# lesliegaga/GPT-SoVITS

Hardware: AMD Instinct MI355X
Metric: synthesised audio sec/sec (1/RTF), v2 pipeline (higher is better)
Workload: dtype f16

## Files before the change

### gpt-sovits_amd/csrc/conv_pair.hip

```cpp
#include <stdlib.h>

#include <algorithm>

#include "common.h"

namespace gsv {

namespace {

typedef _Float16 T;
typedef h8 F;
typedef _Float16 T4 __attribute__((ext_vector_type(4)));

__device__ __forceinline__ void mma32p(f16v& acc, const h8& a, const h8& b) { acc = __builtin_amdgcn_mfma_f32_32x32x16_f16(a, b, acc, 0, 0, 0); }
__device__ __forceinline__ h8 lrelu8(h8 v, float s) { h8 t = v * (_Float16)s; return __builtin_elementwise_max(v, t); }
__device__ __forceinline__ T4 lrelu4(T4 v, float s) { T4 t = v * (_Float16)s; return __builtin_elementwise_max(v, t); }

constexpr int ROWS_Y = 288;
constexpr int ROWS_X = 338;

template <int CC, int TAPS, bool ACCU>
__global__ __launch_bounds__(256, CC == 32 ? 2 : 3) void conv_pair_f16_kernel(ConvPairArgs a, int ntiles) {
  constexpr int G = 8, KC = 16, CT = 32, WN = 4, TN = 2, NT = 256;
  constexpr int LDX = CC + G, VPR = CC / G;
  constexpr int XB = (ROWS_X * VPR + NT - 1) / NT;
  constexpr int WPP = CC == 16 ? 2 : 4, NP = WN / WPP;
  constexpr int LDO = CT + 4, PR = TN * 32 * WPP, IPR = CT / 4, NI = PR * IPR / NT;
  extern __shared__ __attribute__((aligned(16))) unsigned char smem[];
  T* xs = (T*)smem;
  T* ys = xs + (size_t)ROWS_X * LDX;
  T* w2s = ys + (size_t)ROWS_Y * LDX;
  float* os = (float*)smem;
  static_assert(PR * LDO * 4 <= (ROWS_X + ROWS_Y) * LDX * 2, "epilogue tile must fit in window + intermediate image");
  const int tid = threadIdx.x, lane = tid & 63, wn = tid >> 6;
  const int r = lane & 31, h = lane >> 5;
  const T* __restrict__ x = a.x;
  const int h2 = (TAPS - 1) / 2, h1 = h2 * a.dil;
  const int rows_win = ROWS_Y + 2 * h1;
  const int total = rows_win * VPR;
  const int ecg = tid % IPR, ec = 4 * ecg;
  const int env = max(0, min(4, CC - ec));
  f4 ebias = (f4){0.f, 0.f, 0.f, 0.f};
  for (int j = 0; j < env; ++j) ebias[j] = a.b2[ec + j];
  f4 b1v[4];
#pragma unroll
  for (int g = 0; g < 4; ++g)
#pragma unroll
    for (int j = 0; j < 4; ++j) { const int c = 8 * g + 4 * h + j; b1v[g][j] = c < CC ? a.b1[c] : 0.f; }
  {
    const int totw = TAPS * CT * VPR;
    for (int v = tid; v < totw; v += NT) {
      const int tap = v / (CT * VPR), rem = v - tap * (CT * VPR);
      const int row = rem / VPR, col = rem - row * VPR;
      F val = {0, 0, 0, 0, 0, 0, 0, 0};
      if (row < CC) val = *(const F*)(a.w2 + (long long)row * TAPS * CC + (long long)tap * CC + col * G);
      *(F*)(w2s + ((size_t)tap * CT + row) * LDX + col * G) = val;
    }
  }
  F w1r[TAPS * (CC / KC)];
#pragma unroll
  for (int tap = 0; tap < TAPS; ++tap)
#pragma unroll
    for (int ks = 0; ks < CC / KC; ++ks) {
      F val = {0, 0, 0, 0, 0, 0, 0, 0};
      if (r < CC) val = *(const F*)(a.w1 + (long long)r * TAPS * CC + (long long)tap * CC + ks * KC + G * h);
      w1r[tap * (CC / KC) + ks] = val;
    }
  auto load_window = [&](int tile, F* regs) {
    const int win_start = tile * 256 - h2 - h1;
#pragma unroll
    for (int i = 0; i < XB; ++i) {
      const int v = min(tid + i * NT, total - 1);
      const int row = v / VPR, col = v - row * VPR;
      const int ti = win_start + row;
      const F val = *(const F*)(x + (long long)min(max(ti, 0), a.T - 1) * a.ldx + col * G);
      regs[i] = (ti >= 0 && ti < a.T) ? val : (F){0, 0, 0, 0, 0, 0, 0, 0};
    }
  };
  auto store_window = [&](const F* regs) {
#pragma unroll
    for (int i = 0; i < XB; ++i) {
      const int v = tid + i * NT;
      if (v < total) {
        const int row = v / VPR, col = v - row * VPR;
        *(F*)(xs + (size_t)row * LDX + col * G) = lrelu8(regs[i], 0.1f);
      }
    }
  };
  int tile = blockIdx.x;
  {
    F first[XB];
    load_window(min(tile, ntiles - 1), first);
    store_window(first);
  }
  __syncthreads();
  for (; tile < ntiles; tile += gridDim.x) {
    const int t0 = tile * 256;
    F nxt[XB];
    load_window(min(tile + (int)gridDim.x, ntiles - 1), nxt);
    T4 rv[NP * NI], yv[ACCU ? NP * NI : 1];
#pragma unroll
    for (int q = 0; q < NP * NI; ++q) {
      const int pass = q / NI, e = q - pass * NI;
      const int t = min(t0 + pass * PR + (tid + e * NT) / IPR, a.T - 1);
      const int cc = min(ec, CC - 4);
      rv[q] = *(const T4*)(x + (long long)t * a.ldx + cc);
      if (ACCU) yv[q] = *(const T4*)(a.y + (long long)t * a.ldy + cc);
    }
    for (int n1 = wn; n1 < ROWS_Y / 32; n1 += WN) {
      f16v acc;
#pragma unroll
      for (int i = 0; i < 16; ++i) acc[i] = 0.f;
#pragma unroll
      for (int tap = 0; tap < TAPS; ++tap) {
        const int shift = tap * a.dil;
#pragma unroll
        for (int ks = 0; ks < CC / KC; ++ks) {
          const int kk = ks * KC + G * h;
          const F bf = *(const F*)(xs + (size_t)(n1 * 32 + r + shift) * LDX + kk);
          mma32p(acc, w1r[tap * (CC / KC) + ks], bf);
        }
      }
      const int row = n1 * 32 + r, t = t0 - h2 + row;
      const bool inside = t >= 0 && t < a.T;
#pragma unroll
      for (int g = 0; g < 4; ++g) {
        const int c0 = 8 * g + 4 * h;
        if (c0 < CC) {
          T4 v = (T4){(T)(acc[4 * g] + b1v[g][0]), (T)(acc[4 * g + 1] + b1v[g][1]), (T)(acc[4 * g + 2] + b1v[g][2]),
                      (T)(acc[4 * g + 3] + b1v[g][3])};
          v = lrelu4(v, 0.1f);
          if (!inside) v = (T4){0, 0, 0, 0};
          *(T4*)(ys + (size_t)row * LDX + c0) = v;
        }
      }
    }
    __syncthreads();
    f16v acc2[TN];
#pragma unroll
    for (int n = 0; n < TN; ++n)
#pragma unroll
      for (int i = 0; i < 16; ++i) acc2[n][i] = 0.f;
    for (int tap = 0; tap < TAPS; ++tap) {
      const T* wb = w2s + (size_t)tap * CT * LDX;
#pragma unroll
      for (int ks = 0; ks < CC / KC; ++ks) {
        const int kk = ks * KC + G * h;
        const F af = *(const F*)(wb + (size_t)r * LDX + kk);
        F bf[TN];
#pragma unroll
        for (int n = 0; n < TN; ++n) bf[n] = *(const F*)(ys + (size_t)((wn * TN + n) * 32 + r + tap) * LDX + kk);
#pragma unroll
        for (int n = 0; n < TN; ++n) mma32p(acc2[n], af, bf[n]);
      }
    }
#pragma unroll
    for (int pass = 0; pass < NP; ++pass) {
      __syncthreads();
      if (wn / WPP == pass) {
#pragma unroll
        for (int n = 0; n < TN; ++n)
#pragma unroll
          for (int g = 0; g < 4; ++g)
            *(f4*)(os + (size_t)(((wn % WPP) * TN + n) * 32 + r) * LDO + 8 * g + 4 * h) =
                (f4){acc2[n][4 * g], acc2[n][4 * g + 1], acc2[n][4 * g + 2], acc2[n][4 * g + 3]};
      }
      __syncthreads();
#pragma unroll
      for (int e = 0; e < NI; ++e) {
        const int q = pass * NI + e;
        const int tl = (tid + e * NT) / IPR;
        const int t = t0 + pass * PR + tl;
        if (!(t < a.T && env > 0)) continue;
        const f4 av = *(const f4*)(os + (size_t)tl * LDO + 4 * ecg);
        float v[4];
#pragma unroll
        for (int j = 0; j < 4; ++j) {
          float u = av[j] + ebias[j];
          u += (float)rv[q][j];
          u *= a.scale;
          if (ACCU) u += (float)yv[q][j];
          v[j] = u;
        }
        T* yp = a.y + (long long)t * a.ldy + ec;
        if (env == 4) *(T4*)yp = (T4){(T)v[0], (T)v[1], (T)v[2], (T)v[3]};
        else for (int j = 0; j < env; ++j) yp[j] = (T)v[j];
      }
    }
    __syncthreads();
    store_window(nxt);
    __syncthreads();
  }
}

template <int CC, int TAPS>
int launch_pair(const ConvPairArgs& a, hipStream_t s) {
  const int ntiles = cdiv(a.T, 256);
  const size_t lds = ((size_t)ROWS_X + ROWS_Y + (size_t)TAPS * 32) * (CC + 8) * 2;
  static const int cap = getenv("GSV_PAIR_PER_CU") ? std::max(1, atoi(getenv("GSV_PAIR_PER_CU"))) : 3;
  const int per_cu = std::max(1, std::min(cap, (int)((156 * 1024) / lds)));
  const int grid = std::min(ntiles, 256 * per_cu);
#define GSV_PAIR(A)                                                                                                        \
  do {                                                                                                                     \
    auto kern = conv_pair_f16_kernel<CC, TAPS, A>;                                                                         \
    static bool set = false;                                                                                               \
    if (!set) { GSV_HIP(hipFuncSetAttribute((const void*)kern, hipFuncAttributeMaxDynamicSharedMemorySize, 160 * 1024)); set = true; } \
    hipLaunchKernelGGL(kern, dim3(grid), dim3(256), lds, s, a, ntiles);                                                    \
  } while (0)
  if (a.accumulate) GSV_PAIR(true);
  else GSV_PAIR(false);
#undef GSV_PAIR
  GSV_HIP(hipGetLastError());
  return GSV_OK;
}

template <int CC>
int launch_pair_taps(const ConvPairArgs& a, hipStream_t s) {
  switch (a.taps) {
    case 3: return launch_pair<CC, 3>(a, s);
    case 5: return launch_pair<CC, 5>(a, s);
    case 7: return launch_pair<CC, 7>(a, s);
    case 9: return launch_pair<CC, 9>(a, s);
    default: return launch_pair<CC, 11>(a, s);
  }
}

}

bool conv_pair_eligible(int dtype, int C, int taps, int dil, int T) {
  static const bool off = getenv("GSV_NO_CONV_PAIR") != nullptr;
  return !off && dtype == GSV_F16 && (C == 16 || C == 32) && (taps & 1) && taps <= 11 && dil >= 1 && ((taps - 1) / 2) * dil <= 25 &&
         T >= 256;
}

int launch_conv_pair(const ConvPairArgs& a, hipStream_t s) {
  GSV_REQUIRE(a.x && a.y && a.w1 && a.w2 && a.b1 && a.b2, "conv_pair: null operand");
  GSV_REQUIRE(conv_pair_eligible(GSV_F16, a.C, a.taps, a.dil, a.T) || getenv("GSV_NO_CONV_PAIR"), "conv_pair: shape C=%d taps=%d dil=%d T=%d not supported",
              a.C, a.taps, a.dil, a.T);
  GSV_REQUIRE(a.ldx % 8 == 0 && a.ldy % 4 == 0 && ((uintptr_t)a.x % 16) == 0 && ((uintptr_t)a.w1 % 16) == 0 && ((uintptr_t)a.w2 % 16) == 0,
              "conv_pair: operands must be 16-byte aligned");
  return a.C == 16 ? launch_pair_taps<16>(a, s) : launch_pair_taps<32>(a, s);
}

}
```

### gpt-sovits_amd/csrc/ops.hip

```cpp
#include "common.h"

namespace gsv {

static thread_local char g_err[1024] = "";
void set_error(const char* fmt, ...) {
  va_list ap;
  va_start(ap, fmt);
  vsnprintf(g_err, sizeof(g_err), fmt, ap);
  va_end(ap);
}
const char* get_error() { return g_err; }

template <typename T> __global__ void convert_kernel(const float* __restrict__ s, T* __restrict__ d, long long n) {
  long long i = (long long)blockIdx.x * blockDim.x + threadIdx.x;
  long long stride = (long long)gridDim.x * blockDim.x;
  for (; i < n; i += stride) d[i] = (T)s[i];
}

int launch_convert(const float* src, void* dst, int dtype, long long n, hipStream_t s) {
  if (n <= 0) return GSV_OK;
  int blocks = (int)((n + 255) / 256);
  if (blocks > 4096) blocks = 4096;
  if (dtype == GSV_F16) hipLaunchKernelGGL(convert_kernel<_Float16>, dim3(blocks), dim3(256), 0, s, src, (_Float16*)dst, n);
  else hipLaunchKernelGGL(convert_kernel<float>, dim3(blocks), dim3(256), 0, s, src, (float*)dst, n);
  GSV_HIP(hipGetLastError());
  return GSV_OK;
}

template <typename TX, typename TR, typename TY>
__global__ void layernorm_kernel(const TX* __restrict__ x, const TR* __restrict__ res, const float* __restrict__ gamma,
                                 const float* __restrict__ beta, TY* __restrict__ y, int rows, int C, float eps) {
  const int lane = threadIdx.x & 63;
  const int row = blockIdx.x * (blockDim.x >> 6) + (threadIdx.x >> 6);
  if (row >= rows) return;
  const TX* xr = x + (long long)row * C;
  const TR* rr = res ? res + (long long)row * C : nullptr;
  if (C <= 512) {
    float v[8];
    float s1 = 0.f;
#pragma unroll
    for (int i = 0; i < 8; ++i) {
      const int c = lane + 64 * i;
      v[i] = c < C ? to_f(xr[c]) + (rr ? to_f(rr[c]) : 0.f) : 0.f;
      s1 += v[i];
    }
    const float mean1 = wave_sum(s1) / (float)C;
    float q1 = 0.f;
#pragma unroll
    for (int i = 0; i < 8; ++i) {
      const float d = (lane + 64 * i < C) ? v[i] - mean1 : 0.f;
      q1 += d * d;
    }
    const float rstd1 = rsqrtf(wave_sum(q1) / (float)C + eps);
    TY* yr1 = y + (long long)row * C;
#pragma unroll
    for (int i = 0; i < 8; ++i) {
      const int c = lane + 64 * i;
      if (c < C) yr1[c] = (TY)((v[i] - mean1) * rstd1 * gamma[c] + beta[c]);
    }
    return;
  }
  float sum = 0.f;
  for (int c = lane; c < C; c += 64) sum += to_f(xr[c]) + (rr ? to_f(rr[c]) : 0.f);
  const float mean = wave_sum(sum) / (float)C;
  float var = 0.f;
  for (int c = lane; c < C; c += 64) {
    float d = to_f(xr[c]) + (rr ? to_f(rr[c]) : 0.f) - mean;
    var += d * d;
  }
  const float rstd = rsqrtf(wave_sum(var) / (float)C + eps);
  TY* yr = y + (long long)row * C;
  for (int c = lane; c < C; c += 64) {
    float v = to_f(xr[c]) + (rr ? to_f(rr[c]) : 0.f);
    yr[c] = (TY)((v - mean) * rstd * gamma[c] + beta[c]);
  }
}

template <typename TX, typename TR, typename TY>
static int ln_launch(const void* x, const void* res, const float* g, const float* b, void* y, int rows, int C, float eps,
                     hipStream_t s) {
  hipLaunchKernelGGL((layernorm_kernel<TX, TR, TY>), dim3(cdiv(rows, 4)), dim3(256), 0, s, (const TX*)x, (const TR*)res,
                     g, b, (TY*)y, rows, C, eps);
  GSV_HIP(hipGetLastError());
  return GSV_OK;
}

int launch_layernorm(int dtype, const void* x, int x_f32, const void* res, int res_f32, const float* gamma,
                     const float* beta, void* y, int y_f32, int rows, int C, float eps, hipStream_t s) {
  if (rows <= 0) return GSV_OK;
  const bool h = dtype == GSV_F16;
  const bool xf = x_f32 || !h, rf = res_f32 || !h, yf = y_f32 || !h;
  if (xf && rf && yf) return ln_launch<float, float, float>(x, res, gamma, beta, y, rows, C, eps, s);
  if (xf && rf && !yf) return ln_launch<float, float, _Float16>(x, res, gamma, beta, y, rows, C, eps, s);
  if (xf && !rf && !yf) return ln_launch<float, _Float16, _Float16>(x, res, gamma, beta, y, rows, C, eps, s);
  if (!xf && !rf && !yf) return ln_launch<_Float16, _Float16, _Float16>(x, res, gamma, beta, y, rows, C, eps, s);
  if (!xf && !rf && yf) return ln_launch<_Float16, _Float16, float>(x, res, gamma, beta, y, rows, C, eps, s);
  if (!xf && rf && !yf) return ln_launch<_Float16, float, _Float16>(x, res, gamma, beta, y, rows, C, eps, s);
  set_error("layernorm: unsupported dtype combination");
  return GSV_ERR_ARG;
}


template <typename T>
__global__ void frame_kernel(const float* __restrict__ x, int n, int flen, int hop, int pad, int ld, int T_out, T* __restrict__ out) {
  const int t = blockIdx.x;
  if (t >= T_out) return;
  for (int k = threadIdx.x; k < ld; k += blockDim.x) {
    float v = 0.f;
    if (k < flen) {
      int i = t * hop + k - pad;
      if (i < 0) i = -i;
      if (i >= n) i = 2 * (n - 1) - i;
      v = (i >= 0 && i < n) ? x[i] : 0.f;
    }
    out[(long long)t * ld + k] = (T)v;
  }
}

__global__ void magnitude_kernel(const float* __restrict__ ri, int T, int bins, float eps, float* __restrict__ spec) {
  __shared__ float tile[32][33];
  const int t0 = blockIdx.x * 32, b0 = blockIdx.y * 32;
  const int tx = threadIdx.x & 31, ty = threadIdx.x >> 5;
  for (int i = ty; i < 32; i += 8) {
    const int t = t0 + i, b = b0 + tx;
    float v = 0.f;
    if (t < T && b < bins) {
      const float re = ri[(long long)t * 2 * bins + b], im = ri[(long long)t * 2 * bins + bins + b];
      v = eps < 0.f ? re * re + im * im : sqrtf(re * re + im * im + eps);
    }
    tile[i][tx] = v;
  }
  __syncthreads();
  for (int i = ty; i < 32; i += 8) {
    const int b = b0 + i, t = t0 + tx;
    if (b < bins && t < T) spec[(long long)b * T + t] = tile[tx][i];
  }
}

__global__ void magnitude_tm_kernel(const float* __restrict__ ri, int T, int bins, int ld, float eps, float* __restrict__ spec) {
  const int b = blockIdx.x * 256 + threadIdx.x, t = blockIdx.y;
  if (b >= ld) return;
  float v = 0.f;
  if (b < bins) {
    const float re = ri[(long long)t * 2 * bins + b], im = ri[(long long)t * 2 * bins + bins + b];
    v = eps < 0.f ? re * re + im * im : sqrtf(re * re + im * im + eps);
  }
  spec[(long long)t * ld + b] = v;
}

__global__ void aff_mix_kernel(const float* __restrict__ x, const float* __restrict__ y, const float* __restrict__ t, long long n,
                               float* __restrict__ out) {
  const long long i = (long long)blockIdx.x * 256 + threadIdx.x;
  if (i < n) { const float a = t[i]; out[i] = x[i] * (1.f + a) + y[i] * (1.f - a); }
}

__global__ __launch_bounds__(1024) void time_mean_kernel(const float* __restrict__ x, int T, int ld, float* __restrict__ out) {
  __shared__ float part[16][64];
  const int c = blockIdx.x * 64 + (threadIdx.x & 63), sl = threadIdx.x >> 6;
  float s = 0.f;
  if (c < ld) for (int t = sl; t < T; t += 16) s += x[(long long)t * ld + c];
  part[sl][threadIdx.x & 63] = s;
  __syncthreads();
  if (sl == 0 && c < ld) {
    float v = 0.f;
    for (int k = 0; k < 16; ++k) v += part[k][threadIdx.x & 63];
    out[c] = v / (float)T;
  }
}

template <typename T>
__global__ void cnorm_stats_kernel(const T* __restrict__ x, int Tn, int C, int slices, float* __restrict__ part ) {
  const int c = blockIdx.x * blockDim.x + threadIdx.x, sl = blockIdx.y;
  if (c >= C) return;
  const int per = (Tn + slices - 1) / slices, t0 = sl * per, t1 = min(Tn, t0 + per);
  float s = 0.f, q = 0.f;
  for (int t = t0; t < t1; ++t) { const float v = to_f(x[(long long)t * C + c]); s += v; q += v * v; }
  part[((long long)sl * 2 + 0) * C + c] = s;
  part[((long long)sl * 2 + 1) * C + c] = q;
}
template <typename T>
__global__ void cnorm_apply_kernel(const T* __restrict__ x, int Tn, int C, int slices, const float* __restrict__ part,
                                   const float* __restrict__ gamma, const float* __restrict__ beta, float eps, int act, T* __restrict__ y) {
  const int c = blockIdx.x * blockDim.x + threadIdx.x;
  if (c >= C) return;
  double s = 0.0, q = 0.0;
  for (int sl = 0; sl < slices; ++sl) { s += part[((long long)sl * 2 + 0) * C + c]; q += part[((long long)sl * 2 + 1) * C + c]; }
  const float mean = (float)(s / Tn);
  const float var = fmaxf((float)(q / Tn - (s / Tn) * (s / Tn)), 0.f);
  const float a = rsqrtf(var + eps) * gamma[c], b = beta[c] - mean * a;
  const int per = (Tn + gridDim.y - 1) / gridDim.y, t0 = blockIdx.y * per, t1 = min(Tn, t0 + per);
  for (int t = t0; t < t1; ++t) y[(long long)t * C + c] = (T)post_act_f(act, to_f(x[(long long)t * C + c]) * a + b);
}

}

extern "C" {
const char* gsv_last_error(void) { return gsv::get_error(); }
int gsv_abi_version(void) { return 1; }
int gsv_init(int device) {
  int n = 0;
  hipError_t e = hipGetDeviceCount(&n);
  if (e != hipSuccess || n <= 0) {
    gsv::set_error("gsv_init: no HIP device (%s)", hipGetErrorString(e));
    return GSV_ERR_HIP;
  }
  if (device < 0 || device >= n) {
    gsv::set_error("gsv_init: device %d out of range (%d devices)", device, n);
    return GSV_ERR_ARG;
  }
  GSV_HIP(hipSetDevice(device));
  hipDeviceProp_t p;
  GSV_HIP(hipGetDeviceProperties(&p, device));
  if (strncmp(p.gcnArchName, "gfx950", 6) != 0) {
    gsv::set_error("gsv_init: device %d is %s, this library is built for gfx950 only", device, p.gcnArchName);
    return GSV_ERR_HIP;
  }
  return GSV_OK;
}

int gsv_op_layernorm(const void* x, const void* res, const float* gamma, const float* beta, void* y, int rows, int C,
                     float eps, int dtype, gsv_stream_t stream) {
  return gsv::launch_layernorm(dtype, x, 0, res, 0, gamma, beta, y, 0, rows, C, eps, (hipStream_t)stream);
}

int gsv_op_flash_attn64(const void* qkv, int T, int heads, float scale, void* vt_scratch, void* out, gsv_stream_t stream) {
  const int inner = heads * 64;
  return gsv::launch_flash_attn64_f16(qkv, 3 * inner, (const _Float16*)qkv + inner, 3 * inner, (const _Float16*)qkv + 2 * inner, 3 * inner,
                                      vt_scratch, T, heads, scale, out, inner, (hipStream_t)stream);
}

int gsv_op_flash_rel96(const void* qkv, int T, int heads, float scale, const float* rel_k, const float* rel_v, void* vt_scratch,
                       void* out, gsv_stream_t stream) {
  const int H = heads * 96;
  return gsv::launch_flash_rel96_f16(qkv, 3 * H, (const _Float16*)qkv + H, 3 * H, (const _Float16*)qkv + 2 * H, 3 * H, vt_scratch, T, heads,
                                     scale, rel_k, rel_v, out, H, (hipStream_t)stream);
}

int gsv_op_conv1d(const gsv_conv_desc* d, int dtype, gsv_stream_t stream) {
  gsv::ConvArgs a;
  a.x = d->x; a.w = d->w; a.bias = d->bias; a.y = d->y; a.res = d->res; a.gate = d->gate;
  a.T_in = d->T_in; a.T_out = d->T_out; a.Cin = d->Cin; a.Cout = d->Cout; a.taps = d->taps;
  a.stride = d->stride; a.dil = d->dil; a.pad = d->pad;
  a.ldx = d->Cin; a.ldw = d->taps * d->Cin;
  a.pre_act = d->pre_act; a.pre_slope = d->pre_slope; a.post_act = d->post_act; a.scale = d->scale;
  a.accumulate = d->accumulate; a.out_f32 = d->out_f32; a.res_f32 = d->out_f32;
  if (d->ups_u > 0) {
    a.ups_u = d->ups_u; a.ups_pad = d->ups_pad; a.ups_cout = d->Cout / d->ups_u;
    a.ldy = a.ups_cout; a.ldr = a.ups_cout;
    a.T_virt = d->T_in + d->taps - 1;
  } else {
    a.ldy = d->Cout; a.ldr = d->Cout;
    a.T_virt = d->T_out;
  }
  if (d->ldx > 0) a.ldx = d->ldx;
  if (d->ldw > 0) a.ldw = d->ldw;
  if (d->ldy > 0) { a.ldy = d->ldy; a.ldr = d->ldy; }
  if (d->ldr > 0) a.ldr = d->ldr;
  if (d->Z > 1) { a.Z = d->Z; a.xz = d->xz; a.wz = d->wz; a.yz = d->yz; a.bz = d->bz; a.rz = d->rz ? d->rz : d->yz; }
  return gsv::launch_conv_gemm(dtype, a, (hipStream_t)stream);
}

int gsv_op_frame(const float* x, int n, int frame_len, int hop, int pad, int ld, int T_out, void* out, int dtype, gsv_stream_t stream) {
  GSV_REQUIRE(x && out && n > 0 && frame_len > 0 && hop > 0 && ld >= frame_len && T_out > 0, "op_frame: bad argument");
  GSV_REQUIRE(pad >= 0 && pad < n, "op_frame: reflect padding %d needs more than %d samples", pad, pad);
  GSV_REQUIRE((long long)(T_out - 1) * hop + frame_len - pad <= (long long)n + pad, "op_frame: frames run past the (padded) signal");
  GSV_REQUIRE(dtype == GSV_F16 || dtype == GSV_F32, "op_frame: bad dtype");
  hipStream_t s = (hipStream_t)stream;
  if (dtype == GSV_F16) hipLaunchKernelGGL(gsv::frame_kernel<_Float16>, dim3(T_out), dim3(256), 0, s, x, n, frame_len, hop, pad, ld, T_out, (_Float16*)out);
  else hipLaunchKernelGGL(gsv::frame_kernel<float>, dim3(T_out), dim3(256), 0, s, x, n, frame_len, hop, pad, ld, T_out, (float*)out);
  GSV_HIP(hipGetLastError());
  return GSV_OK;
}

int gsv_op_magnitude(const float* re_im, int T, int bins, float eps, int frame_ld, float* spec, gsv_stream_t stream) {
  GSV_REQUIRE(re_im && spec && T > 0 && bins > 0, "op_magnitude: bad argument");
  GSV_REQUIRE(frame_ld == 0 || frame_ld >= bins, "op_magnitude: frame_ld %d is smaller than %d bins", frame_ld, bins);
  if (frame_ld == 0)
    hipLaunchKernelGGL(gsv::magnitude_kernel, dim3(gsv::cdiv(T, 32), gsv::cdiv(bins, 32)), dim3(256), 0, (hipStream_t)stream, re_im, T, bins, eps, spec);
  else
    hipLaunchKernelGGL(gsv::magnitude_tm_kernel, dim3(gsv::cdiv(frame_ld, 256), T), dim3(256), 0, (hipStream_t)stream, re_im, T, bins, frame_ld, eps, spec);
  GSV_HIP(hipGetLastError());
  return GSV_OK;
}

int gsv_op_conv_pair(const void* x, const void* w1, const float* b1, const void* w2, const float* b2, void* y, int T, int C, int taps,
                     int dil, float scale, int accumulate, gsv_stream_t stream) {
  GSV_REQUIRE(gsv::conv_pair_eligible(GSV_F16, C, taps, dil, T), "op_conv_pair: C must be 16 or 32, taps odd <= 11, (taps - 1) / 2 * dil <= 25, T >= 256");
  gsv::ConvPairArgs a;
  a.x = (const _Float16*)x; a.w1 = (const _Float16*)w1; a.b1 = b1; a.w2 = (const _Float16*)w2; a.b2 = b2; a.y = (_Float16*)y;
  a.T = T; a.C = C; a.taps = taps; a.dil = dil; a.ldx = C; a.ldy = C; a.scale = scale; a.accumulate = accumulate;
  return gsv::launch_conv_pair(a, (hipStream_t)stream);
}

int gsv_op_aff_mix(const float* x, const float* y, const float* t, long long n, float* out, gsv_stream_t stream) {
  GSV_REQUIRE(x && y && t && out && n > 0, "op_aff_mix: bad argument");
  hipLaunchKernelGGL(gsv::aff_mix_kernel, dim3((unsigned)((n + 255) / 256)), dim3(256), 0, (hipStream_t)stream, x, y, t, n, out);
  GSV_HIP(hipGetLastError());
  return GSV_OK;
}

int gsv_op_time_mean(const float* x, int T, int ld, float* out, gsv_stream_t stream) {
  GSV_REQUIRE(x && out && T > 0 && ld > 0, "op_time_mean: bad argument");
  hipLaunchKernelGGL(gsv::time_mean_kernel, dim3(gsv::cdiv(ld, 64)), dim3(1024), 0, (hipStream_t)stream, x, T, ld, out);
  GSV_HIP(hipGetLastError());
  return GSV_OK;
}

int gsv_op_channel_norm(const void* x, int T, int C, const float* gamma, const float* beta, float eps, int act, float* scratch,
                        void* y, int dtype, gsv_stream_t stream) {
  GSV_REQUIRE(x && y && gamma && beta && scratch && T > 0 && C > 0, "op_channel_norm: bad argument");
  GSV_REQUIRE(dtype == GSV_F16 || dtype == GSV_F32, "op_channel_norm: bad dtype");
  const int slices = 64;
  hipStream_t s = (hipStream_t)stream;
  const dim3 grid(gsv::cdiv(C, 64), slices);
  if (dtype == GSV_F16) {
    hipLaunchKernelGGL(gsv::cnorm_stats_kernel<_Float16>, grid, dim3(64), 0, s, (const _Float16*)x, T, C, slices, scratch);
    hipLaunchKernelGGL(gsv::cnorm_apply_kernel<_Float16>, grid, dim3(64), 0, s, (const _Float16*)x, T, C, slices, scratch, gamma, beta, eps, act, (_Float16*)y);
  } else {
    hipLaunchKernelGGL(gsv::cnorm_stats_kernel<float>, grid, dim3(64), 0, s, (const float*)x, T, C, slices, scratch);
    hipLaunchKernelGGL(gsv::cnorm_apply_kernel<float>, grid, dim3(64), 0, s, (const float*)x, T, C, slices, scratch, gamma, beta, eps, act, (float*)y);
  }
  GSV_HIP(hipGetLastError());
  return GSV_OK;
}
}
```

Measured before the change: 2782.

## Add fused conv-pair kernel for 64-channel HiFiGAN resblocks

Result: faster. 2817, median of 6 (+1.3%).

```diff
diff --git a/gpt-sovits_amd/csrc/conv_pair.hip b/gpt-sovits_amd/csrc/conv_pair.hip
--- a/gpt-sovits_amd/csrc/conv_pair.hip
+++ b/gpt-sovits_amd/csrc/conv_pair.hip
@@ -225,11 +225,237 @@
   }
 }
 
+constexpr int P64_TT = 128;
+constexpr int P64_RY = 160;
+constexpr int P64_RX = 210;
+
+template <int TAPS, int NW, bool ACCU>
+__global__ __launch_bounds__(64 * NW) void conv_pair64_f16_kernel(ConvPairArgs a, int ntiles) {
+  constexpr int CC = 64, G = 8, KC = 16, NT = 64 * NW, KS = CC / KC;
+  constexpr int WC = NW / 2, TN = 4 / WC;
+  constexpr int LDX = CC + G, VPR = CC / G;
+  constexpr int XB = (P64_RX * VPR + NT - 1) / NT;
+  constexpr int LDO = CC + 4, IPR = CC / 4, NI = P64_TT * IPR / NT;
+  static_assert(P64_TT * LDO * 4 <= (162 + P64_RY) * LDX * 2, "epilogue tile must fit in the smallest window + intermediate image");
+  extern __shared__ __attribute__((aligned(16))) unsigned char smem[];
+  const int h2 = (TAPS - 1) / 2, h1 = h2 * a.dil;
+  const int rows_win = P64_RY + 2 * h1;
+  T* xs = (T*)smem;
+  T* ys = xs + (size_t)rows_win * LDX;
+  T* w2s = ys + (size_t)P64_RY * LDX;
+  float* b1s = (float*)(w2s + (size_t)TAPS * CC * LDX);
+  float* os = (float*)smem;
+  const int tid = threadIdx.x, lane = tid & 63, wave = tid >> 6;
+  const int wm = wave & 1, wc = wave >> 1;
+  const int r = lane & 31, h = lane >> 5;
+  const T* __restrict__ x = a.x;
+  const int total = rows_win * VPR;
+  const int ecg = tid % IPR, ec = 4 * ecg;
+  f4 ebias;
+#pragma unroll
+  for (int j = 0; j < 4; ++j) ebias[j] = a.b2[ec + j];
+  {
+    const int totw = TAPS * CC * VPR;
+    for (int v = tid; v < totw; v += NT) {
+      const int tap = v / (CC * VPR), rem = v - tap * (CC * VPR);
+      const int row = rem / VPR, col = rem - row * VPR;
+      *(F*)(w2s + ((size_t)tap * CC + row) * LDX + col * G) = *(const F*)(a.w2 + (long long)row * TAPS * CC + (long long)tap * CC + col * G);
+    }
+    if (tid < CC) b1s[tid] = a.b1[tid];
+  }
+  F w1r[TAPS * KS];
+#pragma unroll
+  for (int tap = 0; tap < TAPS; ++tap)
+#pragma unroll
+    for (int ks = 0; ks < KS; ++ks)
+      w1r[tap * KS + ks] = *(const F*)(a.w1 + (long long)(wm * 32 + r) * TAPS * CC + (long long)tap * CC + ks * KC + G * h);
+  auto load_window = [&](int tile, F* regs) {
+    const int win_start = tile * P64_TT - h2 - h1;
+#pragma unroll
+    for (int i = 0; i < XB; ++i) {
+      const int v = min(tid + i * NT, total - 1);
+      const int row = v / VPR, col = v - row * VPR;
+      const int ti = win_start + row;
+      const F val = *(const F*)(x + (long long)min(max(ti, 0), a.T - 1) * a.ldx + col * G);
+      regs[i] = (ti >= 0 && ti < a.T) ? val : (F){0, 0, 0, 0, 0, 0, 0, 0};
+    }
+  };
+  auto store_window = [&](const F* regs) {
+#pragma unroll
+    for (int i = 0; i < XB; ++i) {
+      const int v = tid + i * NT;
+      if (v < total) {
+        const int row = v / VPR, col = v - row * VPR;
+        *(F*)(xs + (size_t)row * LDX + col * G) = lrelu8(regs[i], 0.1f);
+      }
+    }
+  };
+  int tile = blockIdx.x;
+  {
+    F first[XB];
+    load_window(min(tile, ntiles - 1), first);
+    store_window(first);
+  }
+  __syncthreads();
+  for (; tile < ntiles; tile += gridDim.x) {
+    const int t0 = tile * P64_TT;
+    F nxt[XB];
+    load_window(min(tile + (int)gridDim.x, ntiles - 1), nxt);
+    for (int n1 = wc; n1 < P64_RY / 32; n1 += WC) {
+      f16v acc;
+#pragma unroll
+      for (int i = 0; i < 16; ++i) acc[i] = 0.f;
+      const T* xb = xs + (size_t)(n1 * 32 + r) * LDX + G * h;
+      if constexpr (NW == 4) {
+        F bb[2][KS];
+#pragma unroll
+        for (int ks = 0; ks < KS; ++ks) bb[0][ks] = *(const F*)(xb + ks * KC);
+#pragma unroll
+        for (int tap = 0; tap < TAPS; ++tap) {
+          if (tap + 1 < TAPS) {
+#pragma unroll
+            for (int ks = 0; ks < KS; ++ks) bb[(tap + 1) & 1][ks] = *(const F*)(xb + (size_t)(tap + 1) * a.dil * LDX + ks * KC);
+          }
+          __builtin_amdgcn_sched_barrier(0);
+#pragma unroll
+          for (int ks = 0; ks < KS; ++ks) mma32p(acc, w1r[tap * KS + ks], bb[tap & 1][ks]);
+        }
+      } else {
+#pragma unroll
+        for (int tap = 0; tap < TAPS; ++tap) {
+          const int shift = tap * a.dil;
+#pragma unroll
+          for (int ks = 0; ks < KS; ++ks) mma32p(acc, w1r[tap * KS + ks], *(const F*)(xb + (size_t)shift * LDX + ks * KC));
+        }
+      }
+      const int row = n1 * 32 + r, t = t0 - h2 + row;
+      const bool inside = t >= 0 && t < a.T;
+#pragma unroll
+      for (int g = 0; g < 4; ++g) {
+        const int c0 = wm * 32 + 8 * g + 4 * h;
+        const f4 bv = *(const f4*)(b1s + c0);
+        T4 v = (T4){(T)(acc[4 * g] + bv[0]), (T)(acc[4 * g + 1] + bv[1]), (T)(acc[4 * g + 2] + bv[2]), (T)(acc[4 * g + 3] + bv[3])};
+        v = lrelu4(v, 0.1f);
+        if (!inside) v = (T4){0, 0, 0, 0};
+        *(T4*)(ys + (size_t)row * LDX + c0) = v;
+      }
+    }
+    T4 rv[NI], yv[ACCU ? NI : 1];
+#pragma unroll
+    for (int e = 0; e < NI; ++e) {
+      const int t = min(t0 + (tid + e * NT) / IPR, a.T - 1);
+      rv[e] = *(const T4*)(x + (long long)t * a.ldx + ec);
+      if (ACCU) yv[e] = *(const T4*)(a.y + (long long)t * a.ldy + ec);
+    }
+    __syncthreads();
+    f16v acc2[TN];
+#pragma unroll
+    for (int n = 0; n < TN; ++n)
+#pragma unroll
+      for (int i = 0; i < 16; ++i) acc2[n][i] = 0.f;
+    const T* wb = w2s + (size_t)(wm * 32 + r) * LDX + G * h;
+    const T* yb = ys + (size_t)(wc * TN * 32 + r) * LDX + G * h;
+    if constexpr (NW == 4) {
+      F ab[2][KS], bb[2][KS][TN];
+      auto load = [&](int tap, F* af, F (*bf)[TN]) {
+#pragma unroll
+        for (int ks = 0; ks < KS; ++ks) {
+          af[ks] = *(const F*)(wb + (size_t)tap * CC * LDX + ks * KC);
+#pragma unroll
+          for (int n = 0; n < TN; ++n) bf[ks][n] = *(const F*)(yb + (size_t)(n * 32 + tap) * LDX + ks * KC);
+        }
+      };
+      load(0, ab[0], bb[0]);
+#pragma unroll
+      for (int tap = 0; tap < TAPS; ++tap) {
+        if (tap + 1 < TAPS) load(tap + 1, ab[(tap + 1) & 1], bb[(tap + 1) & 1]);
+        __builtin_amdgcn_sched_barrier(0);
+#pragma unroll
+        for (int ks = 0; ks < KS; ++ks)
+#pragma unroll
+          for (int n = 0; n < TN; ++n) mma32p(acc2[n], ab[tap & 1][ks], bb[tap & 1][ks][n]);
+      }
+    } else {
+      for (int tap = 0; tap < TAPS; ++tap) {
+#pragma unroll
+        for (int ks = 0; ks < KS; ++ks) {
+          const F af = *(const F*)(wb + (size_t)tap * CC * LDX + ks * KC);
+          F bf[TN];
+#pragma unroll
+          for (int n = 0; n < TN; ++n) bf[n] = *(const F*)(yb + (size_t)(n * 32 + tap) * LDX + ks * KC);
+#pragma unroll
+          for (int n = 0; n < TN; ++n) mma32p(acc2[n], af, bf[n]);
+        }
+      }
+    }
+    __syncthreads();
+#pragma unroll
+    for (int n = 0; n < TN; ++n)
+#pragma unroll
+      for (int g = 0; g < 4; ++g)
+        *(f4*)(os + (size_t)((wc * TN + n) * 32 + r) * LDO + wm * 32 + 8 * g + 4 * h) =
+            (f4){acc2[n][4 * g], acc2[n][4 * g + 1], acc2[n][4 * g + 2], acc2[n][4 * g + 3]};
+    __syncthreads();
+#pragma unroll
+    for (int e = 0; e < NI; ++e) {
+      const int tl = (tid + e * NT) / IPR;
+      const int t = t0 + tl;
+      if (t >= a.T) continue;
+      const f4 av = *(const f4*)(os + (size_t)tl * LDO + 4 * ecg);
+      float v[4];
+#pragma unroll
+      for (int j = 0; j < 4; ++j) {
+        float u = av[j] + ebias[j];
+        u += (float)rv[e][j];
+        u *= a.scale;
+        if (ACCU) u += (float)yv[e][j];
+        v[j] = u;
+      }
+      *(T4*)(a.y + (long long)t * a.ldy + ec) = (T4){(T)v[0], (T)v[1], (T)v[2], (T)v[3]};
+    }
+    __syncthreads();
+    store_window(nxt);
+    __syncthreads();
+  }
+}
+
+template <int TAPS>
+int launch_pair64(const ConvPairArgs& a, hipStream_t s) {
+  const int ntiles = cdiv(a.T, P64_TT);
+  const int h1 = (TAPS - 1) / 2 * a.dil;
+  const size_t lds = ((size_t)P64_RY + 2 * h1 + P64_RY + (size_t)TAPS * 64) * (64 + 8) * 2 + 64 * 4;
+  const int grid = std::min(ntiles, 256);
+  constexpr int NW = TAPS <= 7 ? 8 : 4;
+#define GSV_PAIR64(A)                                                                                                      \
+  do {                                                                                                                     \
+    auto kern = conv_pair64_f16_kernel<TAPS, NW, A>;                                                                       \
+    static bool set = false;                                                                                               \
+    if (!set) { GSV_HIP(hipFuncSetAttribute((const void*)kern, hipFuncAttributeMaxDynamicSharedMemorySize, 160 * 1024)); set = true; } \
+    hipLaunchKernelGGL(kern, dim3(grid), dim3(64 * NW), lds, s, a, ntiles);                                                    \
+  } while (0)
+  if (a.accumulate) GSV_PAIR64(true);
+  else GSV_PAIR64(false);
+#undef GSV_PAIR64
+  GSV_HIP(hipGetLastError());
+  return GSV_OK;
+}
+
+int launch_pair64_taps(const ConvPairArgs& a, hipStream_t s) {
+  switch (a.taps) {
+    case 3: return launch_pair64<3>(a, s);
+    case 5: return launch_pair64<5>(a, s);
+    case 7: return launch_pair64<7>(a, s);
+    case 9: return launch_pair64<9>(a, s);
+    default: return launch_pair64<11>(a, s);
+  }
+}
+
 }
 
 bool conv_pair_eligible(int dtype, int C, int taps, int dil, int T) {
   static const bool off = getenv("GSV_NO_CONV_PAIR") != nullptr;
-  return !off && dtype == GSV_F16 && (C == 16 || C == 32) && (taps & 1) && taps <= 11 && dil >= 1 && ((taps - 1) / 2) * dil <= 25 &&
+  static const bool off64 = getenv("GSV_NO_CONV_PAIR64") != nullptr;
+  return !off && dtype == GSV_F16 && (C == 16 || C == 32 || (C == 64 && !off64)) && (taps & 1) && taps <= 11 && dil >= 1 && ((taps - 1) / 2) * dil <= 25 &&
          T >= 256;
 }
 
@@ -239,6 +465,7 @@
               a.C, a.taps, a.dil, a.T);
   GSV_REQUIRE(a.ldx % 8 == 0 && a.ldy % 4 == 0 && ((uintptr_t)a.x % 16) == 0 && ((uintptr_t)a.w1 % 16) == 0 && ((uintptr_t)a.w2 % 16) == 0,
               "conv_pair: operands must be 16-byte aligned");
+  if (a.C == 64) return launch_pair64_taps(a, s);
   return a.C == 16 ? launch_pair_taps<16>(a, s) : launch_pair_taps<32>(a, s);
 }
 
diff --git a/gpt-sovits_amd/csrc/ops.hip b/gpt-sovits_amd/csrc/ops.hip
--- a/gpt-sovits_amd/csrc/ops.hip
+++ b/gpt-sovits_amd/csrc/ops.hip
@@ -285,7 +285,7 @@
 
 int gsv_op_conv_pair(const void* x, const void* w1, const float* b1, const void* w2, const float* b2, void* y, int T, int C, int taps,
                      int dil, float scale, int accumulate, gsv_stream_t stream) {
-  GSV_REQUIRE(gsv::conv_pair_eligible(GSV_F16, C, taps, dil, T), "op_conv_pair: C must be 16 or 32, taps odd <= 11, (taps - 1) / 2 * dil <= 25, T >= 256");
+  GSV_REQUIRE(gsv::conv_pair_eligible(GSV_F16, C, taps, dil, T), "op_conv_pair: C must be 16, 32 or 64, taps odd <= 11, (taps - 1) / 2 * dil <= 25, T >= 256");
   gsv::ConvPairArgs a;
   a.x = (const _Float16*)x; a.w1 = (const _Float16*)w1; a.b1 = b1; a.w2 = (const _Float16*)w2; a.b2 = b2; a.y = (_Float16*)y;
   a.T = T; a.C = C; a.taps = taps; a.dil = dil; a.ldx = C; a.ldy = C; a.scale = scale; a.accumulate = accumulate;
```
